# vigorbird/ORB_SLAM2_comment

Measured on AMD Instinct MI355X. Metric: frames/sec ORB extract+match, KITTI 1241×376 @1000 feat; HBM GB/s vs peak, higher is better.
Workload: dtype u8; 1 GPU; configs[1]+[2]+[3]: a global batch of 512 synthetic 1241x376 u8 frames per step, 512 per GPU, resident in HBM as (last, cur) pairs; per step ORB extract (nFeatures=1000, 8-level pyramid) of every frame + device-resident SearchByProjection(CurrentFrame, LastFrame, th=15, mono; projection prologue included) for every pair; monocular handles: mvImagePyramid[0] on demand (orbhip_extractor_set_lazy_lev; handles_per_gpu=3, stage_gates=0, global_batch=512, nfeatures=1000, levels=8, parallelism=pair-sharded x1

## Files before the change

### orb_slam2_comment_amd/csrc/orbhip_extractor.hip

```cpp
#include "orbhip_internal.h"
#include "rbrief_pattern.h"

#include <cfloat>
#include <cmath>
#include <ctime>
#include <mutex>
#include <new>
#include <vector>

namespace orbhip {

static thread_local char g_err[512] = "";
void set_error(const char *fmt, ...)
{
    va_list ap;
    va_start(ap, fmt);
    vsnprintf(g_err, sizeof(g_err), fmt, ap);
    va_end(ap);
}

__device__ __forceinline__ void xcd_remap(int &unit, int &frame)
{
    const unsigned T = gridDim.x * gridDim.y, lin = blockIdx.y * gridDim.x + blockIdx.x;
    const unsigned q = T >> 3, r = T & 7, x = lin & 7;
// ... 171 lines not shown
#pragma unroll
            for (int k = 0; k < 4; ++k) {
                const uint32_t h0 = udot2(__builtin_amdgcn_perm(w0h, w0l, sel[k]), alv[k], 0);
                const uint32_t h1 = udot2(__builtin_amdgcn_perm(w1h, w1l, sel[k]), alv[k], 0);
                const uint32_t v = (uint32_t)(((__mul24(b0, (int)(h0 >> 4)) >> 16) + (__mul24(b1, (int)(h1 >> 4)) >> 16) + 2) >> 2) & 0xffu;
                acc |= v << (8 * k);
            }
            out[r] = acc & vmask;
        }
    } else {
#pragma unroll
        for (int r = 0; r < kPyrRows; ++r) {
            const uint8_t *S0 = sroi + (uint32_t)__mul24((int)yt[r].x, P.pitch), *S1 = sroi + (uint32_t)__mul24((int)yt[r].y, P.pitch);
            uint32_t acc = 0;
#pragma unroll
            for (int k = 0; k < 4; ++k)
                acc |= resize_px(S0, S1, sxk[k], (int)(alv[k] & 0xffff), (int)(alv[k] >> 16), yt[r].z, yt[r].w) << (8 * k);
            out[r] = acc & vmask;
        }
    }
#pragma unroll
    for (int r = 0; r < kPyrRows; ++r) {
        const int py = rq * kPyrRows + r;
        if (py < L.prows) *reinterpret_cast<uint32_t *>(dst + (uint32_t)__mul24(py, L.pitch) + pw * 4) = out[r];
    }
}

typedef uint32_t u32x4_t __attribute__((ext_vector_type(4)));
__device__ __forceinline__ uint32_t mulhi24_s(uint32_t a, uint32_t sb)
{
    uint32_t r;
    asm("v_mul_hi_u32_u24 %0, %2, %1" : "=v"(r) : "v"(a), "s"(sb));
    return r;
}
__device__ __forceinline__ PyrRow load_row_rec(const PyrRow *rows, int py)
{
    const u32x4_t raw = *reinterpret_cast<const __attribute__((address_space(4))) u32x4_t *>(reinterpret_cast<uintptr_t>(rows + py));
    return __builtin_bit_cast(PyrRow, raw);
}

__device__ __forceinline__ bool pyr_unit(const PyrLevelTab &T, int unit, int &rg, int &col)
{
    rg = T.nchunks == 1 ? unit : (int)__umulhi((uint32_t)unit, T.rcp_chunks);
    const int c = unit - rg * T.nchunks;
    const int lane = threadIdx.x & 63;
    col = c * T.chunk_w + lane;
    return lane < T.chunk_w && col < T.words;
}

__device__ __forceinline__ void pyr_copy_rows(const PyrLevelTab &T, int unit, const uint8_t *__restrict__ src, int stride,
                                              uint8_t *__restrict__ dplane)
{
    int rg, g;
    if (!pyr_unit(T, unit, rg, g)) return;
    const PyrCopyCol C = reinterpret_cast<const PyrCopyCol *>(T.col)[g];
    const uint32_t base = T.lo[g];
    uint4 win[kPyrRows];
#pragma unroll
    for (int r = 0; r < kPyrRows; ++r) {
        const int py = min(rg * kPyrRows + r, T.prows - 1);
        const int sy = reflect101(py - kEdge, T.src_h);
        __builtin_memcpy(&win[r], src + (size_t)((uint32_t)sy * (uint32_t)stride) + base, 16);
    }
#pragma unroll
    for (int r = 0; r < kPyrRows; ++r) {
        const int py = rg * kPyrRows + r;
        if (py >= T.prows) break;
        uint4 o;
        o.x = __builtin_amdgcn_perm(win[r].y, win[r].x, C.selA[0]) | __builtin_amdgcn_perm(win[r].w, win[r].z, C.selB[0]);
        o.y = __builtin_amdgcn_perm(win[r].y, win[r].x, C.selA[1]) | __builtin_amdgcn_perm(win[r].w, win[r].z, C.selB[1]);
        o.z = __builtin_amdgcn_perm(win[r].y, win[r].x, C.selA[2]) | __builtin_amdgcn_perm(win[r].w, win[r].z, C.selB[2]);
        o.w = __builtin_amdgcn_perm(win[r].y, win[r].x, C.selA[3]) | __builtin_amdgcn_perm(win[r].w, win[r].z, C.selB[3]);
        *reinterpret_cast<uint4 *>(dplane + (size_t)((uint32_t)py * (uint32_t)T.pitch) + (uint32_t)g * 16u) = o;
    }
}

__device__ __forceinline__ void pyr_hfilter(unsigned long long w, const PyrCol &C, uint32_t (&h)[4])
{
    const uint32_t wl = (uint32_t)w, wh = (uint32_t)(w >> 32);
#pragma unroll
    for (int k = 0; k < 4; ++k) h[k] = udot2(__builtin_amdgcn_perm(wh, wl, C.sel[k]), C.alv[k], 0) & ~15u;
}

__device__ __forceinline__ void pyr_resize_rows(const PyrLevelTab &T, int unit, const uint8_t *__restrict__ sroi, int spitch,
                                                uint8_t *__restrict__ dplane)
{
    int rg, pw;
    if (!pyr_unit(T, unit, rg, pw)) return;
    const PyrCol C = reinterpret_cast<const PyrCol *>(T.col)[pw];
    const uint32_t lo = T.lo[pw];
    PyrRow R[kPyrRows];
    unsigned long long w0[kPyrRows], w1[kPyrRows];
#pragma unroll
    for (int r = 0; r < kPyrRows; ++r) {
        R[r] = load_row_rec(T.row, min(rg * kPyrRows + r, T.prows - 1));
        w0[r] = 0;
        if (!(r > 0 && R[r].s0 == R[r - 1].s1))
            __builtin_memcpy(&w0[r], sroi + (size_t)((uint32_t)R[r].s0 * (uint32_t)spitch) + lo, 8);
        __builtin_memcpy(&w1[r], sroi + (size_t)((uint32_t)R[r].s1 * (uint32_t)spitch) + lo, 8);
    }
    uint32_t ha[4], hb[4];
#pragma unroll
    for (int r = 0; r < kPyrRows; ++r) {
        if (r > 0 && R[r].s0 == R[r - 1].s1) {
#pragma unroll
            for (int k = 0; k < 4; ++k) ha[k] = hb[k];
        } else {
            pyr_hfilter(w0[r], C, ha);
        }
        pyr_hfilter(w1[r], C, hb);
        uint32_t acc = 0;
#pragma unroll
        for (int k = 0; k < 4; ++k) {
            const uint32_t v = (mulhi24_s(ha[k], R[r].B0) + mulhi24_s(hb[k], R[r].B1) + 2u) >> 2;
            acc |= v << (8 * k);
        }
        const int py = rg * kPyrRows + r;
        if (py < T.prows) *reinterpret_cast<uint32_t *>(dplane + (size_t)((uint32_t)py * (uint32_t)T.pitch) + (uint32_t)pw * 4u) = acc;
    }
}

__global__ __launch_bounds__(256) void k_pyr_base(const uint8_t *__restrict__ images, int stride, size_t frame_stride,
                                                  uint8_t *__restrict__ pyr, uint32_t frame_bytes, PyrLevelTab T0,
                                                  PyrLevelTab T1, int nb0, int *__restrict__ status)
{
    int bx, fr;
    xcd_remap(bx, fr);
    if (status && bx == 0 && threadIdx.x == 0) status[fr] = 0;
    const int wave = __builtin_amdgcn_readfirstlane((int)(threadIdx.x >> 6));
    const uint8_t *src = images + (size_t)fr * frame_stride;
    uint8_t *frame = pyr + (size_t)fr * frame_bytes;
    if (bx < nb0) {
        const int unit = bx * 4 + wave;
        if (unit < T0.units) pyr_copy_rows(T0, unit, src, stride, frame + T0.plane_off);
    } else {
        const int unit = (bx - nb0) * 4 + wave;
        if (unit < T1.units) pyr_resize_rows(T1, unit, src, stride, frame + T1.plane_off);
    }
}

__global__ __launch_bounds__(256) void k_pyr_rows(uint8_t *__restrict__ pyr, uint32_t frame_bytes, PyrLevelTab T)
{
    int bx, fr;
    xcd_remap(bx, fr);
    const int unit = bx * 4 + __builtin_amdgcn_readfirstlane((int)(threadIdx.x >> 6));
    if (unit >= T.units) return;
    uint8_t *frame = pyr + (size_t)fr * frame_bytes;
    pyr_resize_rows(T, unit, frame + T.src_off, T.src_pitch, frame + T.plane_off);
}

constexpr int kSubMax = 72;
constexpr int kFastStageU = 12;
constexpr int kFastLdsPerCu = 160 * 1024;
constexpr int kFastLdsGranule = 1280;
constexpr int kFastLead = 1;

__device__ __forceinline__ int min3i(int a, int b, int c) { return min(min(a, b), c); }
__device__ __forceinline__ int max3i(int a, int b, int c) { return max(max(a, b), c); }
__device__ __forceinline__ int lane_prefix(unsigned long long m)
{
    return __builtin_amdgcn_mbcnt_hi((unsigned)(m >> 32), __builtin_amdgcn_mbcnt_lo((unsigned)m, 0));
}

typedef unsigned short u16x2_v __attribute__((ext_vector_type(2)));
__device__ __forceinline__ u16x2_v as_u16x2(uint32_t v) { return __builtin_bit_cast(u16x2_v, v); }
__device__ __forceinline__ uint32_t as_u32(u16x2_v v) { return __builtin_bit_cast(uint32_t, v); }
__device__ __forceinline__ uint32_t mulu24(uint32_t a, uint32_t b)
{
    uint32_t r;
    asm("v_mul_u32_u24 %0, %1, %2" : "=v"(r) : "v"(a), "v"(b));
    return r;
}
__device__ __forceinline__ int madi24(int a, int b, int c)
{
    int r;
    asm("v_mad_i32_i24 %0, %1, %2, %3" : "=v"(r) : "v"(a), "v"(b), "v"(c));
    return r;
}
__device__ __forceinline__ uint32_t mulu24_s(uint32_t a, uint32_t sb)
{
    uint32_t r;
    asm("v_mul_u32_u24 %0, %2, %1" : "=v"(r) : "v"(a), "s"(sb));
    return r;
}
__device__ __forceinline__ int madi24_s(int a, int sb, int c)
{
    int r;
    asm("v_mad_i32_i24 %0, %1, %2, %3" : "=v"(r) : "v"(a), "s"(sb), "v"(c));
    return r;
}
__device__ __forceinline__ int add_lane_bit(int x, unsigned long long mask)
{
    int r;
    asm("v_addc_co_u32 %0, vcc, 0, %1, %2" : "=v"(r) : "v"(x), "s"(mask) : "vcc");
    return r;
}

#ifdef ORBHIP_DEVTOOLS
__device__ unsigned long long g_fast_stamps[8];
#endif
__device__ __forceinline__ unsigned long long stamp_now()
{
    unsigned long long t;
    __builtin_amdgcn_sched_barrier(0);
    asm volatile("s_memtime %0\n\ts_waitcnt lgkmcnt(0)" : "=s"(t) :: "memory");
    __builtin_amdgcn_sched_barrier(0);
    return t;
}

#ifndef ORBHIP_FAST_WAVES
#define ORBHIP_FAST_WAVES 8
#endif
template <int SW, bool STAMPS = false>
__global__ __launch_bounds__(64) __attribute__((amdgpu_waves_per_eu(ORBHIP_FAST_WAVES, ORBHIP_FAST_WAVES))) void k_fast_cells(const uint8_t *__restrict__ pyr, const FastCell *__restrict__ cells,
                                                    int *__restrict__ cell_cnt, uint32_t *__restrict__ cell_kp,
                                                    FastParams P, const uint8_t *__restrict__ images, size_t frame_stride)
{
    extern __shared__ uint32_t lds[];
    constexpr int SB = SW * 4;
    constexpr int SS = SB - 8;
// ... 822 lines not shown
    }
    m10 = wave_reduce_add(m10);
    m01 = wave_reduce_add(m01);
    const float angle = fast_atan2_deg((float)m01, (float)m10);
    const float factorPI = (float)(3.14159265358979323846 / 180.f);
    float a, bsn;
    det_sincos(__fmul_rn(angle, factorPI), &a, &bsn);
    __builtin_amdgcn_wave_barrier();
    const uint32_t *hd = reinterpret_cast<const uint32_t *>(hs);
    auto round18 = [](float t) -> int {
        return (int)(__float_as_uint(__fadd_rn(t, 12582912.0f)) - (0x4B400000u - 18u));
    };
    uint32_t vw0, vw1, vw2, vw3, vx0, vx1, vx2, vx3;
    asm("v_mov_b32 %0, %1" : "=v"(vw0) : "s"(w01)); asm("v_mov_b32 %0, %1" : "=v"(vx0) : "s"(w01 ^ w0h));
    asm("v_mov_b32 %0, %1" : "=v"(vw1) : "s"(w23)); asm("v_mov_b32 %0, %1" : "=v"(vx1) : "s"(w23 ^ w12));
    asm("v_mov_b32 %0, %1" : "=v"(vw2) : "s"(w45)); asm("v_mov_b32 %0, %1" : "=v"(vx2) : "s"(w45 ^ w34));
    asm("v_mov_b32 %0, %1" : "=v"(vw3) : "s"(w6l)); asm("v_mov_b32 %0, %1" : "=v"(vx3) : "s"(w6l ^ w56));
    auto blurred = [&](int R, int C) -> int {
        const uint32_t *p = hd + madi24(R >> 1, kHGroups * 4, C);
        const uint32_t d0 = p[0], d1 = p[kHGroups * 4], d2 = p[2 * kHGroups * 4], d3 = p[3 * kHGroups * 4];
        const uint32_t om = 0u - (uint32_t)(R & 1);
        const uint32_t acc = udot2(d0, vw0 ^ (om & vx0), udot2(d1, vw1 ^ (om & vx1), udot2(d2, vw2 ^ (om & vx2),
                                   udot2(d3, vw3 ^ (om & vx3), 32768u))));
        return min((int)(acc >> 16), 255);
    };
    unsigned long long bits[4];
    int t0v[4], t1v[4];
#pragma unroll
    for (int j = 0; j < 4; ++j) {
        const float px0 = pat[j].x, py0 = pat[j].y, px1 = pat[j].z, py1 = pat[j].w;
        const int r0 = round18(__fadd_rn(__fmul_rn(px0, bsn), __fmul_rn(py0, a)));
        const int c0 = round18(__fsub_rn(__fmul_rn(px0, a), __fmul_rn(py0, bsn)));
        const int r1 = round18(__fadd_rn(__fmul_rn(px1, bsn), __fmul_rn(py1, a)));
        const int c1 = round18(__fsub_rn(__fmul_rn(px1, a), __fmul_rn(py1, bsn)));
        t0v[j] = blurred(r0, c0);
        t1v[j] = blurred(r1, c1);
    }
#pragma unroll
    for (int j = 0; j < 4; ++j) bits[j] = __ballot(t0v[j] < t1v[j]);
    if (lane < 4) {
        unsigned long long v = lane == 0 ? bits[0] : lane == 1 ? bits[1] : lane == 2 ? bits[2] : bits[3];
        reinterpret_cast<unsigned long long *>(out_desc + ((size_t)b * cap + oidx) * 32)[lane] = v;
    }
    if (lane == 0) {
        orbhip_keypoint kp;
        float fx = (float)kx, fy = (float)ky;
        const float scale = G.lv[level].scale;
        if (level != 0) { fx = __fmul_rn(fx, scale); fy = __fmul_rn(fy, scale); }
        kp.x = fx; kp.y = fy; kp.size = (float)G.lv[level].patch; kp.angle = angle; kp.response = (float)resp;
        kp.octave = level; kp.class_id = -1;
        out_kp[(size_t)b * cap + oidx] = kp;
    }
  }
}

__global__ void k_zero_status(int *status, int n)
{
    int i = blockIdx.x * blockDim.x + threadIdx.x;
    if (i < n) status[i] = 0;
}

}

using namespace orbhip;

#ifdef ORBHIP_DEVTOOLS
#define ORBHIP_STAGE_MASK(e) ((e)->stage_mask)
#else
#define ORBHIP_STAGE_MASK(e) 31
#endif

static int cv_round(double v) { return (int)lrint(v); }

static void drop_graph(orbhip_extractor *e)
{
    if (e->graph_exec) (void)hipGraphExecDestroy(e->graph_exec);
    e->graph_exec = nullptr; e->graph_batch = 0; e->graph_cap = 0;
}
static void free_geometry(orbhip_extractor *e)
{
    drop_graph(e);
    (void)hipFree(e->d_cells); (void)hipFree(e->d_cells2); (void)hipFree(e->d_tiles); (void)hipFree(e->d_pyrtab);
    e->d_cells = nullptr; e->d_cells2 = nullptr; e->d_tiles = nullptr; e->d_pyrtab = nullptr;
    e->bound = false;
}
static void free_batch(orbhip_extractor *e)
{
    drop_graph(e);
    (void)hipFree(e->d_pyr); (void)hipFree(e->d_blur); (void)hipFree(e->d_cell_cnt); (void)hipFree(e->d_cell_kp);
    (void)hipFree(e->d_keys); (void)hipFree(e->d_knode); (void)hipFree(e->d_sel); (void)hipFree(e->d_sel_cnt); (void)hipFree(e->d_status);
    e->d_pyr = e->d_blur = nullptr; e->d_cell_cnt = nullptr; e->d_cell_kp = nullptr; e->d_keys = nullptr;
    e->d_knode = nullptr; e->d_sel = nullptr; e->d_sel_cnt = nullptr; e->d_status = nullptr;
    e->batch_cap = 0;
    e->blur_valid = false;
}

static void host_resize_coef(int d, double scale, int slen, bool clamp_both, int &s0, int &s1, int &c0, int &c1)
{
#pragma clang fp contract(off)
    const double fd = ((double)d + 0.5) * scale;
    float f = (float)(fd - 0.5);
    int s = (int)floorf(f);
    f = f - (float)s;
    if (clamp_both) {
        s0 = s < 0 ? 0 : (s < slen ? s : slen - 1);
        s1 = s + 1 < 0 ? 0 : (s + 1 < slen ? s + 1 : slen - 1);
    } else {
        if (s < 0) { f = 0.f; s = 0; }
        if (s >= slen - 1) { f = 0.f; s = slen - 1; }
        s0 = s; s1 = s + 1;
    }
    const float g = 1.f - f;
    c0 = (int)lrintf(g * 2048.f);
    c1 = (int)lrintf(f * 2048.f);
}
static int host_reflect101(int p, int len)
{
    if (p < 0) p = -p;
    if (p >= len) p = 2 * (len - 1) - p;
    return p;
}
static void pyr_chunks(PyrLevelTab &T, int rows_per_unit)
{
    T.nchunks = (T.words + 63) / 64;
    T.chunk_w = (T.words + T.nchunks - 1) / T.nchunks;
    T.rcp_chunks = T.nchunks > 1 ? (uint32_t)(((1ull << 32) + (unsigned)T.nchunks - 1) / (unsigned)T.nchunks) : 0u;
    T.units = ((T.prows + rows_per_unit - 1) / rows_per_unit) * T.nchunks;
}

static int build_pyr_tables(orbhip_extractor *e)
{
    const PyrGeom &G = e->G;
    std::vector<uint8_t> blob;
    auto put = [&blob](const void *p, size_t n) {
        const size_t at = (blob.size() + 63) & ~(size_t)63;
        blob.resize(at + n);
        memcpy(blob.data() + at, p, n);
        return at;
    };
    size_t off_row[ORBHIP_MAX_LEVELS] = {0}, off_col[ORBHIP_MAX_LEVELS] = {0}, off_lo[ORBHIP_MAX_LEVELS] = {0};
    for (int l = 0; l < G.nlevels; ++l) {
        const LevelGeom &L = G.lv[l];
        PyrLevelTab &T = e->ptab[l];
        memset(&T, 0, sizeof(T));
        T.prows = L.prows; T.pitch = L.pitch; T.plane_off = L.plane_off;
        e->ptab_rows[l] = false;
        if (l == 0) {
            T.words = L.pitch >> 4;
            T.src_h = L.h;
            std::vector<PyrCopyCol> col(T.words);
            std::vector<uint32_t> lo(T.words);
            for (int g = 0; g < T.words; ++g) {
                int rk[16], base = 1 << 30;
                for (int k = 0; k < 16; ++k) {
                    const int x = g * 16 - kPadL + k;
                    rk[k] = (x >= -kEdge && x < L.w + kEdge) ? host_reflect101(x, L.w) : -1;
                    if (rk[k] >= 0) base = std::min(base, rk[k]);
                }
                if (base == (1 << 30)) base = 0;
                base = std::min(base, L.w - 16);
                lo[g] = (uint32_t)base;
                for (int j = 0; j < 4; ++j) {
                    uint32_t a = 0, b = 0;
                    for (int k = 0; k < 4; ++k) {
                        const int idx = rk[4 * j + k] < 0 ? -1 : rk[4 * j + k] - base;
                        a |= (uint32_t)((idx >= 0 && idx < 8) ? idx : 0x0c) << (8 * k);
                        b |= (uint32_t)((idx >= 8 && idx < 16) ? idx - 8 : 0x0c) << (8 * k);
                    }
                    col[g].selA[j] = a; col[g].selB[j] = b;
                }
            }
            pyr_chunks(T, kPyrRows);
            off_col[l] = put(col.data(), col.size() * sizeof(PyrCopyCol));
            off_lo[l] = put(lo.data(), lo.size() * sizeof(uint32_t));
            e->ptab_rows[l] = true;
            continue;
        }
        const LevelGeom &P = G.lv[l - 1];
        const double sx = 1. / ((double)L.w / P.w), sy = 1. / ((double)L.h / P.h);
        T.words = (kPadL + L.w + kEdge + 3) >> 2;
        T.src_h = P.h; T.src_pitch = P.pitch;
        T.src_off = P.plane_off + (unsigned)(kEdge * P.pitch + kPadL);
        std::vector<PyrCol> col(T.words);
        std::vector<uint32_t> lo(T.words);
        bool ok = P.w >= 8;
        for (int pw = 0; pw < T.words && ok; ++pw) {
            int sxk[4], a0[4], a1[4], lo_ = 1 << 30, hi_ = -1;
            bool valid[4];
            for (int k = 0; k < 4; ++k) {
                const int x = pw * 4 - kPadL + k;
                valid[k] = x >= -kEdge && x < L.w + kEdge;
                sxk[k] = 0; a0[k] = a1[k] = 0;
                if (!valid[k]) continue;
                int s1;
                host_resize_coef(host_reflect101(x, L.w), sx, P.w, false, sxk[k], s1, a0[k], a1[k]);
                lo_ = std::min(lo_, sxk[k]); hi_ = std::max(hi_, sxk[k]);
            }
            if (hi_ < 0) { lo_ = 0; hi_ = 0; }
            if (hi_ - lo_ > 6) { ok = false; break; }
            lo_ = std::min(lo_, P.w - 8);
            lo[pw] = (uint32_t)lo_;
            for (int k = 0; k < 4; ++k) {
                if (!valid[k]) { col[pw].sel[k] = 0x0c0c0c0cu; col[pw].alv[k] = 0; continue; }
                const int rel = sxk[k] - lo_;
                int rel1 = rel + 1;
                if (sxk[k] + 1 > P.w - 1) { rel1 = rel; if (a1[k] != 0) ok = false; }
                if (rel < 0 || rel1 > 7) ok = false;
                col[pw].sel[k] = 0x0c000c00u | (uint32_t)rel | ((uint32_t)rel1 << 16);
                col[pw].alv[k] = (uint32_t)a0[k] | ((uint32_t)a1[k] << 16);
            }
        }
        if (!ok) continue;
        std::vector<PyrRow> row(L.prows);
        for (int py = 0; py < L.prows; ++py) {
            int s0, s1, b0, b1;
            host_resize_coef(host_reflect101(py - kEdge, L.h), sy, P.h, true, s0, s1, b0, b1);
            row[py].s0 = s0; row[py].s1 = s1; row[py].B0 = (uint32_t)b0 << 12; row[py].B1 = (uint32_t)b1 << 12;
        }
        pyr_chunks(T, kPyrRows);
        off_row[l] = put(row.data(), row.size() * sizeof(PyrRow));
        off_col[l] = put(col.data(), col.size() * sizeof(PyrCol));
        off_lo[l] = put(lo.data(), lo.size() * sizeof(uint32_t));
        e->ptab_rows[l] = true;
    }
    ORBHIP_HIP_CHECK(hipMalloc(&e->d_pyrtab, blob.size() + 64));
    ORBHIP_HIP_CHECK(hipMemcpyAsync(e->d_pyrtab, blob.data(), blob.size(), hipMemcpyHostToDevice, e->stream));
    ORBHIP_HIP_CHECK(hipStreamSynchronize(e->stream));
    for (int l = 0; l < G.nlevels; ++l) {
        if (!e->ptab_rows[l]) continue;
        PyrLevelTab &T = e->ptab[l];
        T.row = reinterpret_cast<const PyrRow *>(e->d_pyrtab + off_row[l]);
        T.col = e->d_pyrtab + off_col[l];
        T.lo = reinterpret_cast<const uint32_t *>(e->d_pyrtab + off_lo[l]);
    }
    return ORBHIP_OK;
}

static FastCell make_fast_cell(const PyrGeom &G, const CellDesc &c, int img_stride)
{
    const LevelGeom &Lc = G.lv[c.level];
    FastCell f; memset(&f, 0, sizeof(f));
    const int a = kFastLead, gxb = c.x0 - a, sw = c.x1 - c.x0, shh = c.y1 - c.y0;
    if (img_stride > 0 && c.level == 0) {
        f.src_off = (unsigned)(c.y0 * img_stride + gxb - 4);
        f.pitch = (unsigned short)img_stride; f.img = 1;
    } else {
        f.src_off = Lc.plane_off + (unsigned)((kEdge + c.y0) * Lc.pitch + kPadL + gxb - 4);
        f.pitch = (unsigned short)Lc.pitch;
    }
    f.sw = (unsigned char)sw; f.sh = (unsigned char)shh; f.a = (unsigned char)a;
    f.kpx = (short)(c.offx - 4 - a); f.kpy = (short)(c.offy + 3);
    const int dwc = sw - 6, c_lo = a + 7, c_hi = c_lo + dwc;
    const int ngrp = dwc > 0 ? ((c_hi - 1) >> 2) - (c_lo >> 2) + 1 : 1;
    f.magic = ((1u << 18) + ngrp - 1) / ngrp;
    return f;
}

static int bind_geometry(orbhip_extractor *e, int rows, int cols)
{
    if (e->bound && e->G.rows == rows && e->G.cols == cols) return ORBHIP_OK;
    ORBHIP_HIP_CHECK(hipSetDevice(e->device));
    ORBHIP_HIP_CHECK(hipStreamSynchronize(e->stream));
    free_geometry(e);
    free_batch(e);
    PyrGeom &G = e->G;
    memset(&G, 0, sizeof(G));
    G.nlevels = e->nlevels; G.rows = rows; G.cols = cols; G.ini_th = e->iniTh; G.min_th = e->minTh;
    e->cells.clear(); e->tiles.clear();
    unsigned off = 0;
    int kp_base = 0, cand_base = 0, slot_cap = 1;
    for (int l = 0; l < e->nlevels; ++l) {
        LevelGeom &L = G.lv[l];
        const float scale = e->isf[l];
        L.w = cv_round((float)cols * scale);
        L.h = cv_round((float)rows * scale);
        if (L.w < 2 * kEdge + 2 || L.h < 2 * kEdge + 2 || L.w > 4000 || L.h > 4000) {
            set_error("level %d is %dx%d: unsupported (need 40..4000 px per side)", l, L.w, L.h);
            return ORBHIP_E_SIZE;
        }
        L.pitch = (kPadL + L.w + kEdge + 63) & ~63;
        L.prows = L.h + 2 * kEdge;
        L.plane_off = off;
        off += (unsigned)L.pitch * L.prows;
        off = (off + 255u) & ~255u;
        L.maxBX = L.w - kEdge + 3; L.maxBY = L.h - kEdge + 3;
        L.quota = e->nfeat[l];
        L.patch = (int)(kPatchSize * e->sf[l]);
        L.scale = e->sf[l];
        const int minB = kEdge - 3;
        const float width = (float)(L.maxBX - minB), height = (float)(L.maxBY - minB);
        const float W = 30;
        const int nCols = (int)(width / W), nRows = (int)(height / W);
        L.cell_base = (int)e->cells.size();
        if (nCols >= 1 && nRows >= 1) {
            const int wCell = (int)ceilf(width / nCols), hCell = (int)ceilf(height / nRows);
            if (wCell + 6 > kSubMax || hCell + 6 > kSubMax) { set_error("cell too large"); return ORBHIP_E_SIZE; }
            for (int i = 0; i < nRows; ++i) {
                const float iniY = (float)(minB + i * hCell);
                float maxY = iniY + hCell + 6;
                if (iniY >= L.maxBY - 3) continue;
                if (maxY > L.maxBY) maxY = (float)L.maxBY;
                for (int j = 0; j < nCols; ++j) {
                    const float iniX = (float)(minB + j * wCell);
                    float maxX = iniX + wCell + 6;
                    if (iniX >= L.maxBX - 6) continue;
                    if (maxX > L.maxBX) maxX = (float)L.maxBX;
                    CellDesc c;
                    c.level = (short)l; c.x0 = (short)iniX; c.y0 = (short)iniY; c.x1 = (short)maxX; c.y1 = (short)maxY;
                    c.offx = (short)(j * wCell); c.offy = (short)(i * hCell); c.pad = 0;
                    e->cells.push_back(c);
                    int dw = c.x1 - c.x0 - 6, dh = c.y1 - c.y0 - 6;
                    if (dw > 0 && dh > 0) slot_cap = std::max(slot_cap, ((dw + 1) / 2) * ((dh + 1) / 2));
                }
            }
        }
        L.ncells = (int)e->cells.size() - L.cell_base;
        const int bw = L.maxBX - minB, bh = L.maxBY - minB;
// ... 89 lines not shown
{
    if (batch <= e->batch_cap) return ORBHIP_OK;
    ORBHIP_HIP_CHECK(hipStreamSynchronize(e->stream));
    free_batch(e);
    const PyrGeom &G = e->G;
    const size_t B = (size_t)batch;
    ORBHIP_HIP_CHECK(hipMalloc(&e->d_pyr, B * G.frame_bytes));
    ORBHIP_HIP_CHECK(hipMalloc(&e->d_cell_cnt, B * std::max(G.ncells_total, 1) * sizeof(int)));
    ORBHIP_HIP_CHECK(hipMalloc(&e->d_cell_kp, B * std::max(G.ncells_total, 1) * G.slot_cap * sizeof(uint32_t)));
    ORBHIP_HIP_CHECK(hipMalloc(&e->d_keys, B * G.cand_cap_total * sizeof(uint32_t)));
    ORBHIP_HIP_CHECK(hipMalloc(&e->d_knode, B * G.cand_cap_total * sizeof(unsigned short)));
    ORBHIP_HIP_CHECK(hipMalloc(&e->d_sel, B * G.kp_cap_total * sizeof(uint32_t)));
    ORBHIP_HIP_CHECK(hipMalloc(&e->d_sel_cnt, B * ORBHIP_MAX_LEVELS * sizeof(int)));
    ORBHIP_HIP_CHECK(hipMalloc(&e->d_status, B * sizeof(int)));
    e->batch_cap = batch;
    return ORBHIP_OK;
}

static int begin_extraction(orbhip_extractor *e, const uint8_t *d_images, int stride, size_t frame_stride)
{
    e->blur_valid = false;
    const bool lazy = e->lazy_l0 && e->G.nlevels > 1 && e->ptab_rows[1] && stride <= 65535 &&
                      (unsigned long long)e->G.rows * (unsigned long long)stride < (1ull << 31);
    const int want = lazy ? stride : 0;
    if (want != e->cells_stride && !e->cells.empty()) {
        ORBHIP_HIP_CHECK(hipStreamSynchronize(e->stream));
        drop_graph(e);
        for (size_t i = 0; i < e->cells.size(); ++i)
            if (e->cells[i].level == 0) e->cells2[i] = make_fast_cell(e->G, e->cells[i], want);
        ORBHIP_HIP_CHECK(hipMemcpyAsync(e->d_cells2, e->cells2.data(), e->cells2.size() * sizeof(FastCell), hipMemcpyHostToDevice, e->stream));
        ORBHIP_HIP_CHECK(hipStreamSynchronize(e->stream));
    }
    e->cells_stride = want;
    e->l0_in_image = lazy;
    e->l0_valid = !lazy;
    e->src_images = d_images; e->src_stride = stride; e->src_frame_stride = frame_stride;
    return ORBHIP_OK;
}

int orbhip::ensure_level0(orbhip_extractor *e, hipStream_t consumer)
{
    if (!e || !e->bound || e->last_batch <= 0) return ORBHIP_OK;
    ORBHIP_HIP_CHECK(hipSetDevice(e->device));
    if (!e->l0_valid) {
        PyrLevelTab none; memset(&none, 0, sizeof(none));
        const int nb0 = (e->ptab[0].units + 3) / 4;
        hipLaunchKernelGGL(k_pyr_base, dim3(nb0, e->last_batch), dim3(256), 0, e->stream, e->src_images, e->src_stride,
                           e->src_frame_stride, e->d_pyr, e->G.frame_bytes, e->ptab[0], none, nb0, (int *)nullptr);
        ORBHIP_HIP_CHECK(hipGetLastError());
        e->l0_valid = true;
    }
    if (consumer && consumer != e->stream) {
        if (!e->ev_l0) ORBHIP_HIP_CHECK(hipEventCreateWithFlags(&e->ev_l0, hipEventDisableTiming));
        ORBHIP_HIP_CHECK(hipEventRecord(e->ev_l0, e->stream));
        ORBHIP_HIP_CHECK(hipStreamWaitEvent(consumer, e->ev_l0, 0));
    }
    return ORBHIP_OK;
}

static int launch_pipeline(orbhip_extractor *e, const uint8_t *d_images, int batch, int stride,
                           size_t frame_stride, orbhip_keypoint *d_kps, uint8_t *d_desc, int cap,
                           int *d_n, int *d_status, int frame0 = 0)
{
    const PyrGeom &G = e->G;
    hipStream_t s = e->stream;
    uint8_t *const b_pyr = e->d_pyr + (size_t)frame0 * G.frame_bytes;
    int *const b_cell_cnt = e->d_cell_cnt + (size_t)frame0 * std::max(G.ncells_total, 1);
    uint32_t *const b_cell_kp = e->d_cell_kp + (size_t)frame0 * std::max(G.ncells_total, 1) * G.slot_cap;
    uint32_t *const b_keys = e->d_keys + (size_t)frame0 * G.cand_cap_total;
    unsigned short *const b_knode = e->d_knode + (size_t)frame0 * G.cand_cap_total;
    uint32_t *const b_sel = e->d_sel + (size_t)frame0 * G.kp_cap_total;
    int *const b_sel_cnt = e->d_sel_cnt + (size_t)frame0 * ORBHIP_MAX_LEVELS;
    const bool prof = e->profiling;
    hipEvent_t *ev = prof ? &e->ev[(size_t)(e->prof_calls % orbhip_extractor::kProfRing) * orbhip_extractor::kProfEv] : nullptr;
    int *status = d_status ? d_status : e->d_status + frame0;
    const int sm = ORBHIP_STAGE_MASK(e);
    const bool lazy = e->l0_in_image;
    if (!(sm & 1))
        hipLaunchKernelGGL(k_zero_status, dim3((batch + 255) / 256), dim3(256), 0, s, status, batch);
    if (prof) (void)hipEventRecord(ev[0], s);
#define ORBHIP_GATE_IN(st) do { if (e->gate_wait[st]) (void)hipStreamWaitEvent(s, e->gate_wait[st], 0); } while (0)
#define ORBHIP_GATE_OUT(st) do { if (e->gate_rec[st]) (void)hipEventRecord(e->gate_rec[st], s); } while (0)
    ORBHIP_GATE_IN(0);
    if (sm & 1) {
        const bool l1_rows = G.nlevels > 1 && e->ptab_rows[1];
        PyrLevelTab T1 = e->ptab[1];
        if (!l1_rows) memset(&T1, 0, sizeof(T1));
        const int nb0 = lazy ? 0 : (e->ptab[0].units + 3) / 4, nb1 = (T1.units + 3) / 4;
        hipLaunchKernelGGL(k_pyr_base, dim3(nb0 + nb1, batch), dim3(256), 0, s, d_images, stride, frame_stride, b_pyr,
                           G.frame_bytes, e->ptab[0], T1, nb0, status);
        for (int l = l1_rows ? 2 : 1; l < G.nlevels; ++l) {
            if (e->ptab_rows[l]) {
                hipLaunchKernelGGL(k_pyr_rows, dim3((e->ptab[l].units + 3) / 4, batch), dim3(256), 0, s, b_pyr, G.frame_bytes, e->ptab[l]);
                continue;
            }
            const LevelGeom &Ll = G.lv[l];
            int nl = (Ll.pitch >> 2) * ((Ll.prows + kPyrRows - 1) / kPyrRows);
            const LevelGeom &Pl = G.lv[l - 1];
            const ResizeScale RS = {1. / ((double)Ll.w / Pl.w), 1. / ((double)Ll.h / Pl.h)};
            hipLaunchKernelGGL(k_pyr_resize, dim3((nl + 255) / 256, batch), dim3(256), 0, s, b_pyr, G, l, RS);
        }
    }
    ORBHIP_GATE_OUT(0);
    if (prof) (void)hipEventRecord(ev[1], s);
    ORBHIP_GATE_IN(1);
    if (G.ncells_total > 0 && (sm & 2)) {
        const dim3 grid(G.ncells_total, batch);
        const size_t lb = (size_t)e->fast_lds_bytes;
        FastParams P = e->fast_params;
        P.rcp_cells = (uint32_t)(((1ull << 32) + (unsigned)G.ncells_total - 1) / (unsigned)G.ncells_total);
        if ((unsigned long long)G.ncells_total * G.ncells_total * (unsigned long long)batch >= (1ull << 32)) {
            set_error("batch too large for the FAST kernel's work mapping"); return ORBHIP_E_SIZE;
        }
#define ORBHIP_FAST2(SWv) hipLaunchKernelGGL(k_fast_cells<SWv>, grid, dim3(64), lb, s, b_pyr, e->d_cells2, b_cell_cnt, b_cell_kp, P, d_images, frame_stride)
#ifdef ORBHIP_DEVTOOLS
        P.dev = e->fast_variant;
        if (e->fast_variant == 2 && e->fast_lds.strideW == 11)
            hipLaunchKernelGGL((k_fast_cells<11, true>), grid, dim3(64), lb, s, b_pyr, e->d_cells2, b_cell_cnt, b_cell_kp, P, d_images, frame_stride);
        else
#endif
        switch (e->fast_lds.strideW) {
        case 11: ORBHIP_FAST2(11); break;
        case 13: ORBHIP_FAST2(13); break;
        case 15: ORBHIP_FAST2(15); break;
        case 17: ORBHIP_FAST2(17); break;
        default: ORBHIP_FAST2(21); break;
        }
#undef ORBHIP_FAST2
    }
    ORBHIP_GATE_OUT(1);
    if (prof) (void)hipEventRecord(ev[2], s);
    ORBHIP_GATE_IN(2);
    if (sm & 4) {
        const int ot = e->octree_threads;
#define ORBHIP_OCT(MAXNv, Tv) hipLaunchKernelGGL((k_octree<MAXNv, Tv>), dim3(G.nlevels, batch), dim3(Tv), 0, s, G, b_cell_cnt, b_cell_kp, \
                                                 b_keys, b_knode, b_sel, b_sel_cnt, status)
        if (e->octree_maxn == 512) {
            if (ot == 1024) ORBHIP_OCT(512, 1024); else if (ot == 512) ORBHIP_OCT(512, 512); else ORBHIP_OCT(512, 256);
        } else {
            if (ot == 1024) ORBHIP_OCT(2048, 1024); else if (ot == 512) ORBHIP_OCT(2048, 512); else ORBHIP_OCT(2048, 256);
        }
#undef ORBHIP_OCT
    }
    ORBHIP_GATE_OUT(2);
    if (prof) (void)hipEventRecord(ev[3], s);
    ORBHIP_GATE_IN(3);
    if (sm & 16) {
        const int kDescPerWave = desc_per_wave(G.kp_cap_total, batch, e->num_cus);
        const dim3 grid((G.kp_cap_total + 4 * kDescPerWave - 1) / (4 * kDescPerWave), batch);
        hipLaunchKernelGGL(k_describe_fused, grid, dim3(256), 0, s, b_pyr, G, b_sel, b_sel_cnt, e->d_desc_tab,
                           e->d_patternf, d_kps, d_desc, cap, d_n, status, kDescPerWave, e->blurw,
                           reinterpret_cast<const uint32_t *>(e->d_desc_tab + 768), lazy ? d_images : (const uint8_t *)nullptr, stride,
                           frame_stride);
    }
    ORBHIP_GATE_OUT(3);
#undef ORBHIP_GATE_IN
#undef ORBHIP_GATE_OUT
    if (prof) { (void)hipEventRecord(ev[4], s); e->prof_calls++; }
    e->last_batch = frame0 + batch;
    ORBHIP_HIP_CHECK(hipGetLastError());
    return ORBHIP_OK;
}

extern "C" {

const char *orbhip_last_error(void) { return g_err; }

// ... 552 lines not shown
```

### orb_slam2_comment_amd/csrc/orbhip_internal.h

```cpp
#pragma once
#include "orbhip_common.h"

#include <vector>

struct orbhip_extractor;
namespace orbhip {
struct BlurW { int w[7]; };
struct TileDesc { short level, tx, ty, pad; };
constexpr int kBlurTW = 64, kBlurTH = 58;
struct FastLds {
    int strideW;
    int scoreW;
    int img_words, score_words, list_words;
    int list_cap;
};
struct alignas(32) FastCell {
    uint32_t src_off;
    uint32_t magic;
    unsigned short pitch;
    short kpx, kpy;
    unsigned char sw, sh, a;
    unsigned char img;
    unsigned char pad[14];
};
static_assert(sizeof(FastCell) == 32, "FastCell is one s_load_dwordx8");
struct FastParams {
    uint32_t frame_bytes, rcp_cells;
    int ncells_total, slot_cap, ini_th, min_th, img_words, score_words, list_cap;
    int dev;
};
struct PyrRow { int s0, s1; uint32_t B0, B1; };
struct PyrCol { uint32_t sel[4]; uint32_t alv[4]; };
struct PyrCopyCol { uint32_t selA[4], selB[4]; };
struct PyrLevelTab {
    const PyrRow *row;
    const void *col;
    const uint32_t *lo;
    int words;
    int nchunks, chunk_w;
    uint32_t rcp_chunks;
    int units;
    int prows, pitch;
    unsigned plane_off;
    int src_h, src_pitch;
    unsigned src_off;
};
int ensure_level0(orbhip_extractor *e, hipStream_t consumer);
}

struct orbhip_extractor {
    int nfeatures = 0;
    double scaleFactor = 1.2;
    int nlevels = 8, iniTh = 20, minTh = 7, device = 0;
    float sf[ORBHIP_MAX_LEVELS], isf[ORBHIP_MAX_LEVELS], sig2[ORBHIP_MAX_LEVELS], isig2[ORBHIP_MAX_LEVELS];
    int nfeat[ORBHIP_MAX_LEVELS];
    int umax[orbhip::kHalfPatch + 1];
    orbhip::BlurW blurw;
    hipStream_t stream = nullptr;
    hipStream_t own_stream = nullptr;
    static constexpr int kProfEv = 5;
    static constexpr int kProfRing = 256;
    std::vector<hipEvent_t> ev;
    bool profiling = false;
    long prof_calls = 0;

    bool bound = false;
    orbhip::PyrGeom G;
    std::vector<orbhip::CellDesc> cells;
    std::vector<orbhip::TileDesc> tiles;
    int octree_maxn = 512;
    int octree_threads = 256;
    orbhip::FastLds fast_lds;
    int fast_lds_bytes = 0;
#ifdef ORBHIP_DEVTOOLS
    int stage_mask = 31;
    int fast_variant = 0;
#endif
    orbhip::CellDesc *d_cells = nullptr;
    std::vector<orbhip::FastCell> cells2;
    orbhip::FastCell *d_cells2 = nullptr;
    orbhip::FastParams fast_params;
    int num_cus = 256;
    orbhip::TileDesc *d_tiles = nullptr;
    int *d_desc_tab = nullptr;
    bool blur_valid = false;
    bool lazy_l0 = false;
    bool l0_in_image = false;
    bool l0_valid = true;
    int cells_stride = 0;
    const uint8_t *src_images = nullptr; int src_stride = 0; size_t src_frame_stride = 0;
    hipEvent_t ev_l0 = nullptr;
    hipEvent_t gate_wait[4] = {nullptr, nullptr, nullptr, nullptr}, gate_rec[4] = {nullptr, nullptr, nullptr, nullptr};
    float4 *d_patternf = nullptr;
    uint8_t *d_pyrtab = nullptr;
    orbhip::PyrLevelTab ptab[ORBHIP_MAX_LEVELS];
    bool ptab_rows[ORBHIP_MAX_LEVELS];

    int batch_cap = 0;
    int last_batch = 0;
    uint8_t *d_pyr = nullptr, *d_blur = nullptr;
    int *d_cell_cnt = nullptr;
    uint32_t *d_cell_kp = nullptr;
    uint32_t *d_keys = nullptr;
    unsigned short *d_knode = nullptr;
    uint32_t *d_sel = nullptr;
    int *d_sel_cnt = nullptr;
    int *d_status = nullptr;
    uint8_t *d_img = nullptr; size_t d_img_bytes = 0;
    orbhip_keypoint *d_okp = nullptr; uint8_t *d_odesc = nullptr; int *d_on = nullptr;
    size_t out_slots = 0;
    int out_batch = 0;
    hipGraphExec_t graph_exec = nullptr;
    int graph_batch = 0, graph_cap = 0;
    hipStream_t s_in = nullptr, s_out = nullptr;
    std::vector<hipEvent_t> ev_chunk;
    uint8_t *h_in = nullptr; size_t h_in_bytes = 0;
    uint8_t *h_out = nullptr; size_t h_out_bytes = 0;
};
```

Measured before the change: 291,800 frames/s.

## Fuse pyramid levels 1..N into one tiled kernel with LDS ping-pong halos

Adds a k_pyr_tiles kernel that builds all pyramid levels of a spatial tile in one block. Each level reads its source rows from an LDS ping-pong buffer holding the previous level's footprint instead of global memory. The host planner sizes the tiles, including halo and overlap regions, so each tile computes what the next level needs and writes only the region it owns. This removes the per-level kernel launches and the global round trips between levels, but adds redundant halo computation, __syncthreads barriers and up to 40KB of LDS per block, which can limit occupancy.

```diff
diff --git a/orb_slam2_comment_amd/csrc/orbhip_extractor.hip b/orb_slam2_comment_amd/csrc/orbhip_extractor.hip
--- a/orb_slam2_comment_amd/csrc/orbhip_extractor.hip
+++ b/orb_slam2_comment_amd/csrc/orbhip_extractor.hip
@@ -277,6 +277,29 @@
     for (int k = 0; k < 4; ++k) h[k] = udot2(__builtin_amdgcn_perm(wh, wl, C.sel[k]), C.alv[k], 0) & ~15u;
 }
 
+__device__ __forceinline__ void pyr_filter_rows(const PyrRow (&R)[kPyrRows], const unsigned long long (&w0)[kPyrRows],
+                                                const unsigned long long (&w1)[kPyrRows], const PyrCol &C, uint32_t (&out)[kPyrRows])
+{
+    uint32_t ha[4], hb[4];
+#pragma unroll
+    for (int r = 0; r < kPyrRows; ++r) {
+        if (r > 0 && R[r].s0 == R[r - 1].s1) {
+#pragma unroll
+            for (int k = 0; k < 4; ++k) ha[k] = hb[k];
+        } else {
+            pyr_hfilter(w0[r], C, ha);
+        }
+        pyr_hfilter(w1[r], C, hb);
+        uint32_t acc = 0;
+#pragma unroll
+        for (int k = 0; k < 4; ++k) {
+            const uint32_t v = (mulhi24_s(ha[k], R[r].B0) + mulhi24_s(hb[k], R[r].B1) + 2u) >> 2;
+            acc |= v << (8 * k);
+        }
+        out[r] = acc;
+    }
+}
+
 __device__ __forceinline__ void pyr_resize_rows(const PyrLevelTab &T, int unit, const uint8_t *__restrict__ sroi, int spitch,
                                                 uint8_t *__restrict__ dplane)
 {
@@ -294,24 +317,12 @@
             __builtin_memcpy(&w0[r], sroi + (size_t)((uint32_t)R[r].s0 * (uint32_t)spitch) + lo, 8);
         __builtin_memcpy(&w1[r], sroi + (size_t)((uint32_t)R[r].s1 * (uint32_t)spitch) + lo, 8);
     }
-    uint32_t ha[4], hb[4];
+    uint32_t out[kPyrRows];
+    pyr_filter_rows(R, w0, w1, C, out);
 #pragma unroll
     for (int r = 0; r < kPyrRows; ++r) {
-        if (r > 0 && R[r].s0 == R[r - 1].s1) {
-#pragma unroll
-            for (int k = 0; k < 4; ++k) ha[k] = hb[k];
-        } else {
-            pyr_hfilter(w0[r], C, ha);
-        }
-        pyr_hfilter(w1[r], C, hb);
-        uint32_t acc = 0;
-#pragma unroll
-        for (int k = 0; k < 4; ++k) {
-            const uint32_t v = (mulhi24_s(ha[k], R[r].B0) + mulhi24_s(hb[k], R[r].B1) + 2u) >> 2;
-            acc |= v << (8 * k);
-        }
         const int py = rg * kPyrRows + r;
-        if (py < T.prows) *reinterpret_cast<uint32_t *>(dplane + (size_t)((uint32_t)py * (uint32_t)T.pitch) + (uint32_t)pw * 4u) = acc;
+        if (py < T.prows) *reinterpret_cast<uint32_t *>(dplane + (size_t)((uint32_t)py * (uint32_t)T.pitch) + (uint32_t)pw * 4u) = out[r];
     }
 }
 
@@ -331,6 +342,122 @@
     } else {
         const int unit = (bx - nb0) * 4 + wave;
         if (unit < T1.units) pyr_resize_rows(T1, unit, src, stride, frame + T1.plane_off);
+    }
+}
+
+#ifndef ORBHIP_PYR_TILE_WAVES
+#define ORBHIP_PYR_TILE_WAVES 4
+#endif
+constexpr int kPyrTileWaves = ORBHIP_PYR_TILE_WAVES;
+
+template <bool FROM_LDS>
+__device__ __forceinline__ void pyr_tile_level(const PyrLevelTab &T, const PyrTileRect &R, const PyrTileRect &S,
+                                               const uint8_t *__restrict__ img, int stride, const uint32_t *slds,
+                                               uint32_t *dlds, uint8_t *__restrict__ dplane, int wave)
+{
+    const int ncw = R.cp1 - R.cp0, nrows = R.cr1 - R.cr0;
+    if (ncw <= 0 || nrows <= 0) return;
+    const int nchunks = (ncw + 63) >> 6, chunk_w = (ncw + nchunks - 1) / nchunks;
+    const int nrg = (nrows + kPyrRows - 1) / kPyrRows;
+    const int lane = threadIdx.x & 63;
+    const int dpw = R.fp1 - R.fp0, spw = S.fp1 - S.fp0;
+    int u = 0;
+    for (int c = 0; c < nchunks; ++c) {
+        const int pw = R.cp0 + c * chunk_w + lane;
+        const bool on = lane < chunk_w && pw < R.cp1;
+        const int pwc = on ? pw : R.cp0;
+        const PyrCol C = reinterpret_cast<const PyrCol *>(T.col)[pwc];
+        const uint32_t lo = T.lo[pwc];
+        const bool own_c = on && pw >= R.op0 && pw < R.op1;
+        const bool keep_c = on && pw >= R.fp0 && pw < R.fp1;
+        const int sb = (int)lo + kPadL - 4 * S.fp0;
+        const uint32_t *scol = slds + (sb >> 2);
+        const uint32_t sh = (uint32_t)sb & 3u;
+        for (int rg = 0; rg < nrg; ++rg, ++u) {
+            if ((u & (kPyrTileWaves - 1)) != wave) continue;
+            const int py0 = R.cr0 + rg * kPyrRows;
+            PyrRow Rr[kPyrRows];
+            unsigned long long w0[kPyrRows], w1[kPyrRows];
+#pragma unroll
+            for (int r = 0; r < kPyrRows; ++r) {
+                Rr[r] = load_row_rec(T.row, min(py0 + r, R.cr1 - 1));
+                const bool skip0 = r > 0 && Rr[r].s0 == Rr[r - 1].s1;
+                w0[r] = 0;
+                if (FROM_LDS) {
+                    const uint32_t *p1 = scol + (Rr[r].s1 + kEdge - S.fr0) * spw;
+                    const uint32_t b0 = p1[0], b1 = p1[1], b2 = p1[2];
+                    w1[r] = (unsigned long long)__builtin_amdgcn_alignbyte(b1, b0, sh) |
+                            ((unsigned long long)__builtin_amdgcn_alignbyte(b2, b1, sh) << 32);
+                    if (!skip0) {
+                        const uint32_t *p0 = scol + (Rr[r].s0 + kEdge - S.fr0) * spw;
+                        const uint32_t a0 = p0[0], a1 = p0[1], a2 = p0[2];
+                        w0[r] = (unsigned long long)__builtin_amdgcn_alignbyte(a1, a0, sh) |
+                                ((unsigned long long)__builtin_amdgcn_alignbyte(a2, a1, sh) << 32);
+                    }
+                } else {
+                    if (!skip0) __builtin_memcpy(&w0[r], img + (size_t)((uint32_t)Rr[r].s0 * (uint32_t)stride) + lo, 8);
+                    __builtin_memcpy(&w1[r], img + (size_t)((uint32_t)Rr[r].s1 * (uint32_t)stride) + lo, 8);
+                }
+            }
+            uint32_t out[kPyrRows];
+            pyr_filter_rows(Rr, w0, w1, C, out);
+#pragma unroll
+            for (int r = 0; r < kPyrRows; ++r) {
+                const int py = py0 + r;
+                if (py >= R.cr1) break;
+                if (own_c && py >= R.or0 && py < R.or1)
+                    *reinterpret_cast<uint32_t *>(dplane + (size_t)((uint32_t)py * (uint32_t)T.pitch) + (uint32_t)pw * 4u) = out[r];
+                if (keep_c && py >= R.fr0 && py < R.fr1) dlds[(py - R.fr0) * dpw + (pw - R.fp0)] = out[r];
+            }
+        }
+    }
+}
+
+__device__ __forceinline__ PyrTileRect load_tile_rect(const PyrTileRect *rects, int i)
+{
+    typedef uint32_t u32x8_t __attribute__((ext_vector_type(8)));
+    const u32x8_t raw = *reinterpret_cast<const __attribute__((address_space(4))) u32x8_t *>(reinterpret_cast<uintptr_t>(rects + i));
+    return __builtin_bit_cast(PyrTileRect, raw);
+}
+__device__ __forceinline__ PyrLevelTab load_level_tab(const PyrLevelTab *tabs, int l)
+{
+    struct Raw { uint32_t w[sizeof(PyrLevelTab) / 4]; } raw;
+    const __attribute__((address_space(4))) uint32_t *q =
+        reinterpret_cast<const __attribute__((address_space(4))) uint32_t *>(reinterpret_cast<uintptr_t>(tabs + l));
+#pragma unroll
+    for (int i = 0; i < (int)(sizeof(PyrLevelTab) / 4); ++i) raw.w[i] = q[i];
+    return __builtin_bit_cast(PyrLevelTab, raw);
+}
+
+__global__ __launch_bounds__(64 * kPyrTileWaves) void k_pyr_tiles(const uint8_t *__restrict__ images, int stride, size_t frame_stride,
+                                                   uint8_t *__restrict__ pyr, uint32_t frame_bytes, PyrLevelTab T0, int nb0,
+                                                   PyrTiles P, int *__restrict__ status)
+{
+    extern __shared__ uint32_t pyr_lds[];
+    int bx, fr;
+    xcd_remap(bx, fr);
+    if (status && bx == 0 && threadIdx.x == 0) status[fr] = 0;
+    const int wave = __builtin_amdgcn_readfirstlane((int)(threadIdx.x >> 6));
+    const uint8_t *src = images + (size_t)fr * frame_stride;
+    uint8_t *frame = pyr + (size_t)fr * frame_bytes;
+    if (bx < nb0) {
+        const int unit = bx * kPyrTileWaves + wave;
+        if (unit < T0.units) pyr_copy_rows(T0, unit, src, stride, frame + T0.plane_off);
+        return;
+    }
+    const int tile = bx - nb0;
+    const PyrTileRect *rects = P.rect + tile * P.nlevels;
+    uint32_t *const buf_odd = pyr_lds, *const buf_even = pyr_lds + (P.lds_even >> 2);
+    PyrTileRect S = load_tile_rect(rects, 0);
+    for (int l = 1; l < P.nlevels; ++l) {
+        const PyrLevelTab T = load_level_tab(P.tab, l);
+        const PyrTileRect R = load_tile_rect(rects, l);
+        uint32_t *dl = (l & 1) ? buf_odd : buf_even;
+        const uint32_t *sl = (l & 1) ? buf_even : buf_odd;
+        if (l == 1) pyr_tile_level<false>(T, R, S, src, stride, sl, dl, frame + T.plane_off, wave);
+        else pyr_tile_level<true>(T, R, S, src, stride, sl, dl, frame + T.plane_off, wave);
+        if (l + 1 < P.nlevels) __syncthreads();
+        S = R;
     }
 }
 
@@ -1319,6 +1446,7 @@
     drop_graph(e);
     (void)hipFree(e->d_cells); (void)hipFree(e->d_cells2); (void)hipFree(e->d_tiles); (void)hipFree(e->d_pyrtab);
     e->d_cells = nullptr; e->d_cells2 = nullptr; e->d_tiles = nullptr; e->d_pyrtab = nullptr;
+    memset(&e->ptiles, 0, sizeof(e->ptiles));
     e->bound = false;
 }
 static void free_batch(orbhip_extractor *e)
@@ -1365,6 +1493,92 @@
     T.units = ((T.prows + rows_per_unit - 1) / rows_per_unit) * T.nchunks;
 }
 
+struct PyrSpan { int own0, own1, cmp0, cmp1, fp0, fp1; };
+static void plan_pyr_axis(const PyrGeom &G, const PyrLevelTab *tab, const std::vector<PyrRow> *row,
+                          const std::vector<uint32_t> *lo, bool cols, int n, std::vector<PyrSpan> &sp)
+{
+    const int nl = G.nlevels;
+    sp.assign((size_t)n * nl, PyrSpan{0, 0, 0, 0, 0, 0});
+    for (int i = 0; i < n; ++i)
+        for (int l = nl - 1; l >= 1; --l) {
+            const LevelGeom &L = G.lv[l];
+            auto cut = [&](int k) {
+                if (cols) return k == 0 ? 0 : k == n ? tab[l].words : (kPadL + k * L.w / n) >> 2;
+                return k == 0 ? 0 : k == n ? L.prows : kEdge + k * L.h / n;
+            };
+            PyrSpan &s = sp[(size_t)i * nl + l];
+            s.own0 = cut(i); s.own1 = cut(i + 1);
+            int f0 = 1 << 30, f1 = -1;
+            if (l + 1 < nl) {
+                const PyrSpan &d = sp[(size_t)i * nl + l + 1];
+                for (int q = d.cmp0; q < d.cmp1; ++q) {
+                    if (cols) {
+                        const int b = ((int)lo[l + 1][q] + kPadL) >> 2;
+                        f0 = std::min(f0, b); f1 = std::max(f1, b + 3);
+                    } else {
+                        const PyrRow &R = row[l + 1][q];
+                        f0 = std::min(f0, std::min(R.s0, R.s1) + kEdge); f1 = std::max(f1, std::max(R.s0, R.s1) + kEdge + 1);
+                    }
+                }
+            }
+            if (f0 >= f1) f0 = f1 = 0;
+            s.fp0 = f0; s.fp1 = f1;
+            if (s.own0 >= s.own1) { s.cmp0 = f0; s.cmp1 = f1; }
+            else if (f0 >= f1) { s.cmp0 = s.own0; s.cmp1 = s.own1; }
+            else { s.cmp0 = std::min(s.own0, f0); s.cmp1 = std::max(s.own1, f1); }
+        }
+}
+
+#ifndef ORBHIP_PYR_TILE_W1
+#define ORBHIP_PYR_TILE_W1 64
+#endif
+#ifndef ORBHIP_PYR_TILE_LDS_KB
+#define ORBHIP_PYR_TILE_LDS_KB 40
+#endif
+constexpr int kPyrTileLdsMax = ORBHIP_PYR_TILE_LDS_KB * 1024;
+
+static bool plan_pyr_tiles(const PyrGeom &G, const PyrLevelTab *tab, const std::vector<PyrRow> *row, const std::vector<uint32_t> *lo,
+                           std::vector<PyrTileRect> &rects, int &tx, int &ty, int &lds, unsigned &lds_even)
+{
+    const int nl = G.nlevels;
+    const LevelGeom &D = G.lv[nl - 1];
+    std::vector<PyrSpan> cs, rs;
+    tx = 0;
+    for (int n = 1; n <= 16 && 4 * n <= D.w; ++n) {
+        plan_pyr_axis(G, tab, row, lo, true, n, cs);
+        int mw = 0;
+        for (int i = 0; i < n; ++i) mw = std::max(mw, cs[(size_t)i * nl + 1].cmp1 - cs[(size_t)i * nl + 1].cmp0);
+        if (mw <= ORBHIP_PYR_TILE_W1) { tx = n; break; }
+    }
+    if (!tx) return false;
+    for (int n = 1; n <= 64 && n <= D.h; ++n) {
+        plan_pyr_axis(G, tab, row, lo, false, n, rs);
+        int need[2] = {0, 0};
+        for (int i = 0; i < tx; ++i)
+            for (int j = 0; j < n; ++j)
+                for (int l = 1; l + 1 < nl; ++l) {
+                    const PyrSpan &c = cs[(size_t)i * nl + l], &r = rs[(size_t)j * nl + l];
+                    need[l & 1] = std::max(need[l & 1], 4 * (c.fp1 - c.fp0) * (r.fp1 - r.fp0));
+                }
+        lds_even = (unsigned)((need[1] + 15) & ~15);
+        lds = (int)lds_even + need[0];
+        if (lds > kPyrTileLdsMax) continue;
+        ty = n;
+        rects.assign((size_t)tx * ty * nl, PyrTileRect{});
+        for (int j = 0; j < ty; ++j)
+            for (int i = 0; i < tx; ++i)
+                for (int l = 1; l < nl; ++l) {
+                    const PyrSpan &c = cs[(size_t)i * nl + l], &r = rs[(size_t)j * nl + l];
+                    PyrTileRect &t = rects[((size_t)j * tx + i) * nl + l];
+                    t.cp0 = (short)c.cmp0; t.cp1 = (short)c.cmp1; t.cr0 = (short)r.cmp0; t.cr1 = (short)r.cmp1;
+                    t.op0 = (short)c.own0; t.op1 = (short)c.own1; t.or0 = (short)r.own0; t.or1 = (short)r.own1;
+                    t.fp0 = (short)c.fp0; t.fp1 = (short)c.fp1; t.fr0 = (short)r.fp0; t.fr1 = (short)r.fp1;
+                }
+        return true;
+    }
+    return false;
+}
+
 static int build_pyr_tables(orbhip_extractor *e)
 {
     const PyrGeom &G = e->G;
@@ -1376,6 +1590,8 @@
         return at;
     };
     size_t off_row[ORBHIP_MAX_LEVELS] = {0}, off_col[ORBHIP_MAX_LEVELS] = {0}, off_lo[ORBHIP_MAX_LEVELS] = {0};
+    std::vector<PyrRow> host_row[ORBHIP_MAX_LEVELS];
+    std::vector<uint32_t> host_lo[ORBHIP_MAX_LEVELS];
     for (int l = 0; l < G.nlevels; ++l) {
         const LevelGeom &L = G.lv[l];
         PyrLevelTab &T = e->ptab[l];
@@ -1459,10 +1675,21 @@
         off_col[l] = put(col.data(), col.size() * sizeof(PyrCol));
         off_lo[l] = put(lo.data(), lo.size() * sizeof(uint32_t));
         e->ptab_rows[l] = true;
+        host_row[l] = std::move(row);
+        host_lo[l] = std::move(lo);
+    }
+    bool tiled = G.nlevels > 1;
+    for (int l = 1; l < G.nlevels; ++l) tiled = tiled && e->ptab_rows[l];
+    std::vector<PyrTileRect> rects;
+    int tx = 0, ty = 0, lds = 0;
+    unsigned lds_even = 0;
+    if (tiled) tiled = plan_pyr_tiles(G, e->ptab, host_row, host_lo, rects, tx, ty, lds, lds_even);
+    size_t off_tab = 0, off_rect = 0;
+    if (tiled) {
+        off_tab = put(e->ptab, sizeof(PyrLevelTab) * G.nlevels);
+        off_rect = put(rects.data(), rects.size() * sizeof(PyrTileRect));
     }
     ORBHIP_HIP_CHECK(hipMalloc(&e->d_pyrtab, blob.size() + 64));
-    ORBHIP_HIP_CHECK(hipMemcpyAsync(e->d_pyrtab, blob.data(), blob.size(), hipMemcpyHostToDevice, e->stream));
-    ORBHIP_HIP_CHECK(hipStreamSynchronize(e->stream));
     for (int l = 0; l < G.nlevels; ++l) {
         if (!e->ptab_rows[l]) continue;
         PyrLevelTab &T = e->ptab[l];
@@ -1470,6 +1697,19 @@
         T.col = e->d_pyrtab + off_col[l];
         T.lo = reinterpret_cast<const uint32_t *>(e->d_pyrtab + off_lo[l]);
     }
+    memset(&e->ptiles, 0, sizeof(e->ptiles));
+    e->ptile_lds = 0; e->ptile_tx = e->ptile_ty = 0;
+    if (tiled) {
+        memcpy(blob.data() + off_tab, e->ptab, sizeof(PyrLevelTab) * G.nlevels);
+        e->ptiles.tab = reinterpret_cast<const PyrLevelTab *>(e->d_pyrtab + off_tab);
+        e->ptiles.rect = reinterpret_cast<const PyrTileRect *>(e->d_pyrtab + off_rect);
+        e->ptiles.ntiles = tx * ty;
+        e->ptiles.nlevels = G.nlevels;
+        e->ptiles.lds_even = lds_even;
+        e->ptile_lds = lds; e->ptile_tx = tx; e->ptile_ty = ty;
+    }
+    ORBHIP_HIP_CHECK(hipMemcpyAsync(e->d_pyrtab, blob.data(), blob.size(), hipMemcpyHostToDevice, e->stream));
+    ORBHIP_HIP_CHECK(hipStreamSynchronize(e->stream));
     return ORBHIP_OK;
 }
 
@@ -1725,7 +1965,11 @@
 #define ORBHIP_GATE_IN(st) do { if (e->gate_wait[st]) (void)hipStreamWaitEvent(s, e->gate_wait[st], 0); } while (0)
 #define ORBHIP_GATE_OUT(st) do { if (e->gate_rec[st]) (void)hipEventRecord(e->gate_rec[st], s); } while (0)
     ORBHIP_GATE_IN(0);
-    if (sm & 1) {
+    if ((sm & 1) && e->ptiles.ntiles > 0) {
+        const int nb0 = lazy ? 0 : (e->ptab[0].units + kPyrTileWaves - 1) / kPyrTileWaves;
+        hipLaunchKernelGGL(k_pyr_tiles, dim3(nb0 + e->ptiles.ntiles, batch), dim3(64 * kPyrTileWaves), (size_t)e->ptile_lds, s, d_images, stride,
+                           frame_stride, b_pyr, G.frame_bytes, e->ptab[0], nb0, e->ptiles, status);
+    } else if (sm & 1) {
         const bool l1_rows = G.nlevels > 1 && e->ptab_rows[1];
         PyrLevelTab T1 = e->ptab[1];
         if (!l1_rows) memset(&T1, 0, sizeof(T1));
diff --git a/orb_slam2_comment_amd/csrc/orbhip_internal.h b/orb_slam2_comment_amd/csrc/orbhip_internal.h
--- a/orb_slam2_comment_amd/csrc/orbhip_internal.h
+++ b/orb_slam2_comment_amd/csrc/orbhip_internal.h
@@ -44,6 +44,19 @@
     unsigned plane_off;
     int src_h, src_pitch;
     unsigned src_off;
+};
+struct alignas(32) PyrTileRect {
+    short cp0, cp1, cr0, cr1;
+    short op0, op1, or0, or1;
+    short fp0, fp1, fr0, fr1;
+    short pad[4];
+};
+static_assert(sizeof(PyrTileRect) == 32, "PyrTileRect is one s_load_dwordx8");
+struct PyrTiles {
+    const PyrLevelTab *tab;
+    const PyrTileRect *rect;
+    int ntiles, nlevels;
+    unsigned lds_even;
 };
 int ensure_level0(orbhip_extractor *e, hipStream_t consumer);
 }
@@ -95,6 +108,9 @@
     uint8_t *d_pyrtab = nullptr;
     orbhip::PyrLevelTab ptab[ORBHIP_MAX_LEVELS];
     bool ptab_rows[ORBHIP_MAX_LEVELS];
+    orbhip::PyrTiles ptiles = {};
+    int ptile_lds = 0;
+    int ptile_tx = 0, ptile_ty = 0;
 
     int batch_cap = 0;
     int last_batch = 0;
```

Measured after the change: 256,100 frames/s (median of 2 runs). 0.878x the previous value.
